# TrentMahaffey/NeuralStyleTransferV1

Hardware: AMD Instinct MI355X
Metric: stylized 1080p frames/sec at 1/2/4/8 MI355X; SSIM vs CPU ref (higher is better)
Workload: dtype bf16; 1 GPU; configs[1]: TransformerNet (Johnson) forward, 1920x1080, batch 8 per GPU, bf16 MFMA / fp32 accumulate, io_preset imagenet_255, uint8 frames in/out resident in HBM; global_batch=8, parallelism=frames round-robin over 1 GPU(s), no data-path collective, ranks_per_gpu=1, step_launch=one HIP-graph replay of the captured forward per step

## Files before the change

neuralstyletransferv1_amd/csrc/conv_out9.hip:

```cpp
#include <algorithm>
#include <cstring>

#include "conv_impl.h"

namespace nst {

typedef __attribute__((address_space(3))) uint64_t lds_u64;

template <int CINP, int G, int NW, int ESZ = 2>
struct Out9Cfg {
  static constexpr int KC = CINP * ESZ / 32;
  static constexpr int NCH = CINP * ESZ / 16;
  static constexpr int CPCH = 16 / ESZ;
  static constexpr int EB = CINP * ESZ + 16;
  static constexpr int SW = 32 * G;
  static constexpr int LWS = SW + 8;
  static constexpr int ROWB = LWS * EB;
  static constexpr int WAVE_LDS = 2 * ROWB;
  static constexpr int NBLK = 9 * KC;
  static constexpr int BLK_BYTES = 2 * 27 * 8;
  static constexpr int PART_BYTES = NBLK * BLK_BYTES;
  static constexpr int W_BYTES = 2 * PART_BYTES;
  static constexpr int W_OFF = NW * WAVE_LDS;
  static constexpr int LDS = W_OFF + W_BYTES;
  static constexpr int ITEMS = LWS * NCH;
  static constexpr int IPL = (ITEMS + 63) / 64;
  static constexpr int PPJ = 64 / NCH;
  static_assert(64 % NCH == 0, "a lane keeps one channel chunk");
  static_assert(LDS <= 160 * 1024, "LDS budget");
};

template <typename T, int CINP, int G, int NW, int OUTK, bool TANH, int CLD = CINP>
__global__ __launch_bounds__(64 * NW) void out9_kernel(ConvParams p) {
  constexpr bool SPLIT = IS_SPLIT<T>;
  using TM = std::conditional_t<SPLIT, _Float16, T>;
  using C = Out9Cfg<CINP, G, NW, SPLIT ? 4 : 2>;
  constexpr int KC = C::KC, EB = C::EB;
  __shared__ __attribute__((aligned(16))) char smem[C::LDS];
  const int tid = threadIdx.x, lane = tid & 63;
  const int wave = __builtin_amdgcn_readfirstlane(tid >> 6);

  {
    const uint4* src = (const uint4*)p.wpk;
    uint4* dst = (uint4*)(smem + C::W_OFF);
    for (int i = tid; i < C::W_BYTES / 16; i += 64 * NW) dst[i] = src[i];
  }
  __syncthreads();

  const int item = blockIdx.x * NW + wave;
  if (item >= p.n_work) return;
  const int strips = p.tiles_x, nseg = p.tiles_y;
  const int strip = item % strips;
  const int rest = item / strips;
  const int seg = rest % nseg;
  const int n = rest / nseg;
  const int x0 = strip * C::SW;
  const int o0 = seg * p.seg_len;
  const int L = min(p.seg_len, p.oh - o0);
  if (L <= 0) return;
  const int NV = L + 8;

  const int rho = lane & 31, h = lane >> 5;
  int a_off[9];
  {
    const int k = rho < 27 ? rho / 3 : 0;
    const int c = rho < 27 ? rho - 3 * (rho / 3) : 0;
#pragma unroll
    for (int t = 0; t < 9; ++t) {
      a_off[t] = C::W_OFF + (h * 27 + 3 * ((t - k + 9) % 9) + c) * 8;
      asm volatile("" : "+v"(a_off[t]));
    }
  }
  char* ring = smem + wave * C::WAVE_LDS;
  const int b_lane = rho * EB + 16 * h;
  const int chunk = lane / C::PPJ;
  const int pix_bytes = p.cs * (SPLIT ? 4 : 2);
  const int row_bytes = p.ws * pix_bytes;
  int coloff[C::IPL];
#pragma unroll
  for (int j = 0; j < C::IPL; ++j) {
    const int col = C::PPJ * j + lane % C::PPJ;
    const int sx = map_axis(x0 + p.crop_x - p.pad + col, p.ws, p.axis_mode, p.pre);
    coloff[j] = (col < C::LWS && sx >= 0 && chunk * C::CPCH < CLD) ? sx * pix_bytes + chunk * 16 : -1;
  }
  float2 nm[C::CPCH];
#pragma unroll
  for (int j = 0; j < C::CPCH; ++j)
    nm[j] = chunk * C::CPCH < CLD ? p.in_norm[(size_t)n * p.cs + chunk * C::CPCH + j] : make_float2(0.f, 0.f);
  const char* img = (const char*)p.in + (size_t)n * p.hs * row_bytes;
  const int vy0 = o0 + p.crop_y - p.pad;

  auto row_src = [&](int v) -> int {
    const int sy = map_axis(vy0 + v, p.hs, p.axis_mode, p.pre);
    return sy < 0 ? -1 : sy * row_bytes;
  };
  uint4 raw[C::IPL];
  const __amdgpu_buffer_rsrc_t rs = __builtin_amdgcn_make_buffer_rsrc((void*)img, (short)0, p.hs * row_bytes, 0x00020000);
  constexpr uint32_t OOB = 0x80000000u;
  auto issue = [&](int ro) {
#pragma unroll
    for (int j = 0; j < C::IPL; ++j) {
      const bool ok = ro >= 0 && coloff[j] >= 0;
      raw[j] = __builtin_bit_cast(uint4, __builtin_amdgcn_raw_buffer_load_b128(rs, ok ? (uint32_t)(ro + coloff[j]) : OOB, 0, 0));
    }
  };
  auto store_row = [&](int v, int ro) {
    char* dst = ring + (v & 1) * C::ROWB + (lane % C::PPJ) * EB + chunk * 16;
#pragma unroll
    for (int j = 0; j < C::IPL; ++j) {
      if (C::PPJ * j + lane % C::PPJ < C::LWS) {
        const bool ok = ro >= 0 && coloff[j] >= 0;
        const uint4 v4 = lds_form<T>(norm_chunk<T>(raw[j], nm));
        *(uint4*)(dst + j * C::PPJ * EB) = ok ? v4 : make_uint4(0u, 0u, 0u, 0u);
      }
    }
  };

  const float bias[3] = {p.bias[0], p.bias[1], p.bias[2]};
  float dp[3], dq[3], dri[3], ds[3];
#pragma unroll
  for (int c = 0; c < 3; ++c) {
    const int ch = p.dec_perm[c];
    dp[c] = p.dec_p[ch]; dq[c] = p.dec_q[ch]; dri[c] = 1.0f / p.dec_r[ch]; ds[c] = p.dec_s[ch];
  }
  const int out_bytes = OUTK == OUT_F32_NCHW ? 3 * p.oh * p.ow * 4 : p.oh * p.ow * 3;
  const __amdgpu_buffer_rsrc_t ors = __builtin_amdgcn_make_buffer_rsrc(
      (void*)((char*)p.out + (size_t)n * out_bytes), (short)0, out_bytes, 0x00020000);
  int perm[3];
#pragma unroll
  for (int c = 0; c < 3; ++c) perm[c] = p.dec_perm[c];
  auto emit = [&](const f32x16_t (&acc)[G], int reg, int c, int oy, bool on) {
#pragma unroll
    for (int gi = 0; gi < G; ++gi) {
      const int ox = x0 + gi * 32 + rho;
      const bool ok = on && ox < p.ow;
      float y = acc[gi][reg] + bias[c];
      if constexpr (TANH) y = tanhf(y);
      if constexpr (OUTK == OUT_F32_NCHW) {
        __builtin_amdgcn_raw_buffer_store_b32(__float_as_int(y), ors, ok ? (uint32_t)(((c * p.oh + oy) * p.ow + ox) * 4) : OOB, 0, 0);
      } else {
        const float v = fminf(fmaxf((y + dp[c]) * dq[c] * dri[c] + ds[c], 0.f), 1.f);
        __builtin_amdgcn_raw_buffer_store_b8((uint8_t)(v * 255.0f), ors,
                                             ok ? (uint32_t)((oy * p.ow + ox) * 3 + perm[c]) : OOB, 0, 0);
      }
    }
  };

  f32x16_t acc[G];
#pragma unroll
  for (int gi = 0; gi < G; ++gi)
#pragma unroll
    for (int r = 0; r < 16; ++r) acc[gi][r] = 0.f;

  {
    const int ro0 = row_src(0);
    issue(ro0);
    store_row(0, ro0);
  }
  for (int vb = 0; vb < NV; vb += 9) {
#pragma unroll
    for (int t = 0; t < 9; ++t) {
      const int v = vb + t;
      if (v >= NV) break;
      const bool next = v + 1 < NV;
      const int ro_next = next ? row_src(v + 1) : -1;
      if (next) issue(ro_next);
      const char* rb = ring + (v & 1) * C::ROWB + b_lane;
      const char* ab = smem + a_off[t];
      constexpr int AF = SPLIT ? 2 : 1;
      uint4 av[2][KC][AF], bv[2][KC][G];
      auto ld = [&](int kx, uint4 (&a)[KC][AF], uint4 (&b)[KC][G]) {
#pragma unroll
        for (int kc = 0; kc < KC; ++kc) {
          const uint64_t a0 = *(const volatile lds_u64*)(ab + (kx * KC + kc) * C::BLK_BYTES);
          const uint64_t a1 = *(const volatile lds_u64*)(ab + (kx * KC + kc) * C::BLK_BYTES + C::PART_BYTES);
          if constexpr (SPLIT) {
            a[kc][0] = make_uint4((uint32_t)a0, (uint32_t)(a0 >> 32), (uint32_t)a0, (uint32_t)(a0 >> 32));
            a[kc][AF - 1] = make_uint4((uint32_t)a1, (uint32_t)(a1 >> 32), 0u, 0u);
          } else {
            a[kc][0] = make_uint4((uint32_t)a0, (uint32_t)(a0 >> 32), (uint32_t)a1, (uint32_t)(a1 >> 32));
          }
#pragma unroll
          for (int gi = 0; gi < G; ++gi) b[kc][gi] = *(const uint4*)(rb + (gi * 32 + kx) * EB + kc * 32);
        }
      };
      ld(0, av[0], bv[0]);
#pragma unroll
      for (int kx = 0; kx < 9; ++kx) {
        if (kx + 1 < 9) ld(kx + 1, av[(kx + 1) & 1], bv[(kx + 1) & 1]);
#pragma unroll
        for (int kc = 0; kc < KC; ++kc)
#pragma unroll
          for (int gi = 0; gi < G; ++gi)
#pragma unroll
            for (int f = 0; f < AF; ++f)
              acc[gi] = mfma32x32x16<TM>(av[kx & 1][kc][f], bv[kx & 1][kc][gi], acc[gi]);
        __builtin_amdgcn_sched_barrier(0);
      }
      const int kk = (t + 1) % 9;
#pragma unroll
      for (int c = 0; c < 3; ++c) {
        const int r3 = 3 * kk + c;
        const int reg = (r3 & 3) + 4 * (r3 >> 3), hh = (r3 >> 2) & 1;
        emit(acc, reg, c, o0 + v - 8, v >= 8 && h == hh);
#pragma unroll
        for (int gi = 0; gi < G; ++gi) acc[gi][reg] = (h == hh) ? 0.f : acc[gi][reg];
      }
      if (next) store_row(v + 1, ro_next);
    }
  }
}

template <typename T, int CINP, int G, int NW, int OUTK, bool TANH, int CLD = CINP>
struct Out9Inst {
  using C = Out9Cfg<CINP, G, NW, IS_SPLIT<T> ? 4 : 2>;
  static constexpr auto kernel = out9_kernel<T, CINP, G, NW, OUTK, TANH, CLD>;
  static int cus() {
    static const int v = [] {
      int dev = 0, c = 0;
      if (hipGetDevice(&dev) != hipSuccess || hipDeviceGetAttribute(&c, hipDeviceAttributeMultiprocessorCount, dev) != hipSuccess)
        c = 256;
      return c;
    }();
    return v;
  }
  static void launch(const ConvParams& p0, dim3 grid, hipStream_t st) {
    ConvParams p = p0;
    const int n = (int)grid.y;
    const int strips = (p.ow + C::SW - 1) / C::SW;
    const int slots = cus() * NW;
    int nseg = std::max(1, slots / std::max(1, n * strips));
    nseg = std::min(nseg, std::max(1, p.oh / 16));
    p.seg_len = (p.oh + nseg - 1) / nseg;
    nseg = (p.oh + p.seg_len - 1) / p.seg_len;
    p.tiles_x = strips;
    p.tiles_y = nseg;
    p.n_work = n * nseg * strips;
    const int blocks = (p.n_work + NW - 1) / NW;
    hipLaunchKernelGGL(kernel, dim3(blocks), dim3(64 * NW), 0, st, p);
  }
  static ConvKernelInfo info() {
    ConvKernelInfo k;
    std::memset(&k, 0, sizeof(k));
    k.dtype = dtype_code<T>();
    k.mode = MODE_KYROT;
    k.ks = 9; k.stride = 1; k.cinp = CLD; k.bn = 16;
    k.cinp_k = CLD != CINP ? CINP : 0; k.th = 1; k.tw = C::SW; k.wm = NW; k.wn = 1;
    k.in_kind = IN_ACT; k.out_kind = OUTK;
    k.cpc = C::CPCH; k.nch = C::NCH; k.lds_bytes = C::LDS;
    k.in_esz = IS_SPLIT<T> ? 4 : 0;
    k.wbytes = C::W_BYTES;
    k.part_rows = 1;
    k.tanh_out = TANH ? 1 : 0;
    k.launch = &launch;
    return k;
  }
};

#ifndef NST_OUT9_R_G
#define NST_OUT9_R_G 1
#endif
#ifndef NST_OUT9_R_NW
#define NST_OUT9_R_NW 8
#endif
#ifndef NST_OUT9_J_G
#define NST_OUT9_J_G 3
#endif
#ifndef NST_OUT9_J_NW
#define NST_OUT9_J_NW 8
#endif
#ifndef NST_OUT9_S_G
#define NST_OUT9_S_G 1
#endif
#ifndef NST_OUT9_S_NW
#define NST_OUT9_S_NW 8
#endif
#define E(...) Out9Inst<__VA_ARGS__>::info()
const ConvKernelInfo* conv_table_out9(int* count) {
  static const ConvKernelInfo table[] = {
      E(__bf16, 32, NST_OUT9_J_G, NST_OUT9_J_NW, OUT_U8_NHWC, false),
      E(__bf16, 32, 3, 8, OUT_F32_NCHW, false),
      E(__bf16, 64, NST_OUT9_R_G, NST_OUT9_R_NW, OUT_U8_NHWC, true),
      E(__bf16, 64, NST_OUT9_R_G, NST_OUT9_R_NW, OUT_F32_NCHW, true),
      E(__bf16, 64, NST_OUT9_R_G, NST_OUT9_R_NW, OUT_U8_NHWC, true, 48),
      E(__bf16, 64, NST_OUT9_R_G, NST_OUT9_R_NW, OUT_F32_NCHW, true, 48),
      E(_Float16, 32, 3, 8, OUT_U8_NHWC, false),
      E(_Float16, 32, 3, 8, OUT_F32_NCHW, false),
      E(_Float16, 64, NST_OUT9_R_G, NST_OUT9_R_NW, OUT_U8_NHWC, true),
      E(_Float16, 64, NST_OUT9_R_G, NST_OUT9_R_NW, OUT_F32_NCHW, true),
      E(_Float16, 64, NST_OUT9_R_G, NST_OUT9_R_NW, OUT_U8_NHWC, true, 48),
      E(_Float16, 64, NST_OUT9_R_G, NST_OUT9_R_NW, OUT_F32_NCHW, true, 48),
      E(F32Split, 32, NST_OUT9_S_G, NST_OUT9_S_NW, OUT_U8_NHWC, false),
      E(F32Split, 32, NST_OUT9_S_G, NST_OUT9_S_NW, OUT_F32_NCHW, false),
  };
  *count = (int)(sizeof(table) / sizeof(table[0]));
  return table;
}
#undef E

}
```

Measured before the change: 1615 frames/s.

## Software-pipeline out9 conv: interleave row loads, LDS fills and output stores with MFMAs

New measurement: 1618 frames/s, median of 6. Within noise of the previous version (+0.2%).

```diff
diff --git a/neuralstyletransferv1_amd/csrc/conv_out9.hip b/neuralstyletransferv1_amd/csrc/conv_out9.hip
--- a/neuralstyletransferv1_amd/csrc/conv_out9.hip
+++ b/neuralstyletransferv1_amd/csrc/conv_out9.hip
@@ -1,11 +1,22 @@
 #include <algorithm>
 #include <cstring>
+#include <utility>
 
 #include "conv_impl.h"
 
 namespace nst {
 
 typedef __attribute__((address_space(3))) uint64_t lds_u64;
+
+#ifndef NST_OUT9_PIPE
+#define NST_OUT9_PIPE 1
+#endif
+#ifndef NST_OUT9_PIPE_TANH
+#define NST_OUT9_PIPE_TANH 0
+#endif
+#ifndef NST_OUT9_VPM
+#define NST_OUT9_VPM 8
+#endif
 
 template <int CINP, int G, int NW, int ESZ = 2>
 struct Out9Cfg {
@@ -22,7 +33,8 @@
   static constexpr int PART_BYTES = NBLK * BLK_BYTES;
   static constexpr int W_BYTES = 2 * PART_BYTES;
   static constexpr int W_OFF = NW * WAVE_LDS;
-  static constexpr int LDS = W_OFF + W_BYTES;
+  static constexpr int Z_OFF = W_OFF + W_BYTES;
+  static constexpr int LDS = Z_OFF + ROWB;
   static constexpr int ITEMS = LWS * NCH;
   static constexpr int IPL = (ITEMS + 63) / 64;
   static constexpr int PPJ = 64 / NCH;
@@ -30,12 +42,18 @@
   static_assert(LDS <= 160 * 1024, "LDS budget");
 };
 
+template <int... Ts, typename F>
+__device__ __forceinline__ bool out9_rows(std::integer_sequence<int, Ts...>, F& f) {
+  return (f(std::integral_constant<int, Ts>{}) && ...);
+}
+
 template <typename T, int CINP, int G, int NW, int OUTK, bool TANH, int CLD = CINP>
 __global__ __launch_bounds__(64 * NW) void out9_kernel(ConvParams p) {
   constexpr bool SPLIT = IS_SPLIT<T>;
   using TM = std::conditional_t<SPLIT, _Float16, T>;
   using C = Out9Cfg<CINP, G, NW, SPLIT ? 4 : 2>;
   constexpr int KC = C::KC, EB = C::EB;
+  constexpr bool PIPE = TANH ? NST_OUT9_PIPE_TANH != 0 : NST_OUT9_PIPE != 0;
   __shared__ __attribute__((aligned(16))) char smem[C::LDS];
   const int tid = threadIdx.x, lane = tid & 63;
   const int wave = __builtin_amdgcn_readfirstlane(tid >> 6);
@@ -44,6 +62,8 @@
     const uint4* src = (const uint4*)p.wpk;
     uint4* dst = (uint4*)(smem + C::W_OFF);
     for (int i = tid; i < C::W_BYTES / 16; i += 64 * NW) dst[i] = src[i];
+    uint4* z = (uint4*)(smem + C::Z_OFF);
+    for (int i = tid; i < C::ROWB / 16; i += 64 * NW) z[i] = make_uint4(0u, 0u, 0u, 0u);
   }
   __syncthreads();
 
@@ -97,14 +117,14 @@
   uint4 raw[C::IPL];
   const __amdgpu_buffer_rsrc_t rs = __builtin_amdgcn_make_buffer_rsrc((void*)img, (short)0, p.hs * row_bytes, 0x00020000);
   constexpr uint32_t OOB = 0x80000000u;
-  auto issue = [&](int ro) {
+  [[maybe_unused]] auto issue = [&](int ro) {
 #pragma unroll
     for (int j = 0; j < C::IPL; ++j) {
       const bool ok = ro >= 0 && coloff[j] >= 0;
       raw[j] = __builtin_bit_cast(uint4, __builtin_amdgcn_raw_buffer_load_b128(rs, ok ? (uint32_t)(ro + coloff[j]) : OOB, 0, 0));
     }
   };
-  auto store_row = [&](int v, int ro) {
+  [[maybe_unused]] auto store_row = [&](int v, int ro) {
     char* dst = ring + (v & 1) * C::ROWB + (lane % C::PPJ) * EB + chunk * 16;
 #pragma unroll
     for (int j = 0; j < C::IPL; ++j) {
@@ -129,7 +149,7 @@
   int perm[3];
 #pragma unroll
   for (int c = 0; c < 3; ++c) perm[c] = p.dec_perm[c];
-  auto emit = [&](const f32x16_t (&acc)[G], int reg, int c, int oy, bool on) {
+  [[maybe_unused]] auto emit = [&](const f32x16_t (&acc)[G], int reg, int c, int oy, bool on) {
 #pragma unroll
     for (int gi = 0; gi < G; ++gi) {
       const int ox = x0 + gi * 32 + rho;
@@ -152,6 +172,146 @@
 #pragma unroll
     for (int r = 0; r < 16; ++r) acc[gi][r] = 0.f;
 
+  if constexpr (PIPE) {
+  constexpr int IPL = C::IPL, NS = 3 * G;
+  static_assert(IPL <= 9, "one fill item per tap at most");
+  constexpr uint32_t ESTR = OUTK == OUT_F32_NCHW ? 4 : 3;
+  int fdst[IPL];
+#pragma unroll
+  for (int j = 0; j < IPL; ++j)
+    fdst[j] = coloff[j] >= 0 ? (lane % C::PPJ) * EB + chunk * 16 + j * C::PPJ * EB
+                             : (lane % C::PPJ) * EB + CINP * (SPLIT ? 4 : 2);
+  for (int i = lane * 16; i < C::WAVE_LDS; i += 64 * 16) *(uint4*)(ring + i) = make_uint4(0u, 0u, 0u, 0u);
+  auto fill_item = [&](int j, char* slot) {
+    *(uint4*)(slot + fdst[j]) = lds_form<T>(norm_chunk<T>(raw[j], nm));
+  };
+  uint32_t lcol[IPL];
+#pragma unroll
+  for (int j = 0; j < IPL; ++j) lcol[j] = coloff[j] >= 0 ? (uint32_t)coloff[j] : OOB;
+  auto issue_item = [&](int j, int ro) {
+    const __amdgpu_buffer_rsrc_t rr = __builtin_amdgcn_make_buffer_rsrc((void*)img, (short)0, ro >= 0 ? p.hs * row_bytes : 0, 0x00020000);
+    raw[j] = __builtin_bit_cast(uint4, __builtin_amdgcn_raw_buffer_load_b128(rr, lcol[j], ro >= 0 ? ro : 0, 0));
+  };
+  uint32_t colo[2][3][G];
+#pragma unroll
+  for (int hh = 0; hh < 2; ++hh)
+#pragma unroll
+    for (int c = 0; c < 3; ++c)
+#pragma unroll
+      for (int gi = 0; gi < G; ++gi) {
+        const int ox = x0 + gi * 32 + rho;
+        colo[hh][c][gi] = (ox >= p.ow || h != hh) ? OOB
+                          : OUTK == OUT_F32_NCHW ? (uint32_t)((c * p.oh * p.ow + ox) * 4) : (uint32_t)(ox * 3 + perm[c]);
+      }
+  float pend[3][G];
+  uint32_t prow = 0;
+  __amdgpu_buffer_rsrc_t prs = __builtin_amdgcn_make_buffer_rsrc((void*)((char*)p.out + (size_t)n * out_bytes), (short)0, 0, 0x00020000);
+#pragma unroll
+  for (int c = 0; c < 3; ++c)
+#pragma unroll
+    for (int gi = 0; gi < G; ++gi) pend[c][gi] = 0.f;
+  auto emit_slice = [&](int c, int gi, int kk) {
+    const int r3 = 3 * kk + c;
+    const int hh = (r3 >> 2) & 1;
+    float y = pend[c][gi];
+    if constexpr (TANH) y = tanhf(y);
+    const uint32_t off = colo[hh][c][gi];
+    if constexpr (OUTK == OUT_F32_NCHW) {
+      __builtin_amdgcn_raw_buffer_store_b32(__float_as_int(y), prs, off, prow, 0);
+    } else {
+      const float v = fminf(fmaxf((y + dp[c]) * dq[c] * dri[c] + ds[c], 0.f), 1.f);
+      __builtin_amdgcn_raw_buffer_store_b8((uint8_t)(v * 255.0f), prs, off, prow, 0);
+    }
+  };
+
+  int ro0 = row_src(0), ro1 = row_src(1);
+#pragma unroll
+  for (int j = 0; j < IPL; ++j) issue_item(j, ro0);
+#pragma unroll
+  for (int j = 0; j < IPL; ++j) {
+    fill_item(j, ring);
+    issue_item(j, ro1);
+  }
+  int vb = 0;
+  auto row = [&](auto tc) -> bool {
+      constexpr int t = decltype(tc)::value;
+      const int v = vb + t;
+      if (v >= NV) return false;
+      const int ro2 = v + 2 < NV ? row_src(v + 2) : -1;
+      const char* rb = smem + (ro0 >= 0 ? wave * C::WAVE_LDS + (v & 1) * C::ROWB : C::Z_OFF) + b_lane;
+      char* wb = ring + ((v + 1) & 1) * C::ROWB;
+      const char* ab = smem + a_off[t];
+      constexpr int AF = SPLIT ? 2 : 1;
+      uint4 av[2][KC][AF], bv[2][KC][G];
+      auto ld = [&](int kx, uint4 (&a)[KC][AF], uint4 (&b)[KC][G]) {
+#pragma unroll
+        for (int kc = 0; kc < KC; ++kc) {
+          const uint64_t a0 = *(const volatile lds_u64*)(ab + (kx * KC + kc) * C::BLK_BYTES);
+          const uint64_t a1 = *(const volatile lds_u64*)(ab + (kx * KC + kc) * C::BLK_BYTES + C::PART_BYTES);
+          if constexpr (SPLIT) {
+            a[kc][0] = make_uint4((uint32_t)a0, (uint32_t)(a0 >> 32), (uint32_t)a0, (uint32_t)(a0 >> 32));
+            a[kc][AF - 1] = make_uint4((uint32_t)a1, (uint32_t)(a1 >> 32), 0u, 0u);
+          } else {
+            a[kc][0] = make_uint4((uint32_t)a0, (uint32_t)(a0 >> 32), (uint32_t)a1, (uint32_t)(a1 >> 32));
+          }
+#pragma unroll
+          for (int gi = 0; gi < G; ++gi) b[kc][gi] = *(const uint4*)(rb + (gi * 32 + kx) * EB + kc * 32);
+        }
+      };
+      ld(0, av[0], bv[0]);
+#pragma unroll
+      for (int kx = 0; kx < 9; ++kx) {
+        if (kx + 1 < 9) ld(kx + 1, av[(kx + 1) & 1], bv[(kx + 1) & 1]);
+#pragma unroll
+        for (int j = 0; j < IPL; ++j)
+          if (j * 9 / IPL == kx) {
+            fill_item(j, wb);
+            issue_item(j, ro2);
+          }
+#pragma unroll
+        for (int s = 0; s < NS; ++s)
+          if (s * 9 / NS == kx) emit_slice(s / G, s % G, t);
+#pragma unroll
+        for (int kc = 0; kc < KC; ++kc)
+#pragma unroll
+          for (int gi = 0; gi < G; ++gi)
+#pragma unroll
+            for (int f = 0; f < AF; ++f)
+              acc[gi] = mfma32x32x16<TM>(av[kx & 1][kc][f], bv[kx & 1][kc][gi], acc[gi]);
+        constexpr int NM = KC * G * AF;
+#pragma unroll
+        for (int m = 0; m < NM; ++m) {
+          __builtin_amdgcn_sched_group_barrier(0x008, 1, 0);
+          __builtin_amdgcn_sched_group_barrier(0x100, (KC * (2 + G) + NM - 1) / NM, 0);
+          __builtin_amdgcn_sched_group_barrier(0x002, NST_OUT9_VPM, 0);
+        }
+        __builtin_amdgcn_sched_barrier(0);
+      }
+      const int kk = (t + 1) % 9;
+#pragma unroll
+      for (int c = 0; c < 3; ++c) {
+        const int r3 = 3 * kk + c;
+        const int reg = (r3 & 3) + 4 * (r3 >> 3), hh = (r3 >> 2) & 1;
+#pragma unroll
+        for (int gi = 0; gi < G; ++gi) {
+          pend[c][gi] = acc[gi][reg] + bias[c];
+          acc[gi][reg] = (h == hh) ? 0.f : acc[gi][reg];
+        }
+      }
+      prow = v >= 8 ? (uint32_t)(o0 + v - 8) * (uint32_t)p.ow * ESTR : 0u;
+      prs = __builtin_amdgcn_make_buffer_rsrc((void*)((char*)p.out + (size_t)n * out_bytes), (short)0, v >= 8 ? out_bytes : 0, 0x00020000);
+      ro0 = ro1;
+      ro1 = ro2;
+      return true;
+  };
+  for (; vb < NV; vb += 9)
+    if (!out9_rows(std::make_integer_sequence<int, 9>{}, row)) break;
+  {
+    const int kk = NV % 9;
+#pragma unroll
+    for (int s = 0; s < NS; ++s) emit_slice(s / G, s % G, kk);
+  }
+  } else {
   {
     const int ro0 = row_src(0);
     issue(ro0);
@@ -208,6 +368,7 @@
       }
       if (next) store_row(v + 1, ro_next);
     }
+  }
   }
 }
 
```
